# mfkiwl/msckf_stereo_c

Hardware: AMD Instinct MI355X
Metric: stereo frames/sec/node on EuRoC-shape input; ATE RMSE vs CPU ref (higher is better)
Workload: dtype f64

## Files before the change

msckf_stereo_c_amd/csrc/hip/ekf_kernels.hip:

```cpp
#include <mutex>
#include <type_traits>
#include "ekf_device.h"
#include "chol_block.h"

#define WG 256

__device__ __forceinline__ double wave_sum(double v) {
    for (int off = 32; off > 0; off >>= 1) v += __shfl_xor(v, off);
    return v;
}

__device__ __forceinline__ double block_sum(double v, double *s_red) {
    v = wave_sum(v);
    const int nw = blockDim.x >> 6;
    __syncthreads();
    if ((threadIdx.x & 63) == 0) s_red[threadIdx.x >> 6] = v;
    __syncthreads();
    double t = 0;
    for (int i = 0; i < nw; ++i) t += s_red[i];
    return t;
}

__device__ __forceinline__ void quat_to_rot(const double *q, double *R) {
    const double x = q[0], y = q[1], z = q[2], w = q[3];
    const double a = 2 * w * w - 1, tw = 2 * w;
    R[0] = a + 2 * x * x;        R[1] = tw * z + 2 * x * y;   R[2] = -tw * y + 2 * x * z;
    R[3] = -tw * z + 2 * y * x;  R[4] = a + 2 * y * y;        R[5] = tw * x + 2 * y * z;
    R[6] = tw * y + 2 * z * x;   R[7] = -tw * x + 2 * z * y;  R[8] = a + 2 * z * z;
}
__device__ __forceinline__ void mat3_mul(const double *A, const double *B, double *C) {
    for (int i = 0; i < 3; ++i) for (int j = 0; j < 3; ++j) C[3 * i + j] = A[3 * i] * B[j] + A[3 * i + 1] * B[3 + j] + A[3 * i + 2] * B[6 + j];
}
__device__ __forceinline__ void mat3_vec(const double *A, const double *v, double *o) {
    for (int i = 0; i < 3; ++i) o[i] = A[3 * i] * v[0] + A[3 * i + 1] * v[1] + A[3 * i + 2] * v[2];
}
__device__ __forceinline__ void mat3t_vec(const double *A, const double *v, double *o) {
    for (int i = 0; i < 3; ++i) o[i] = A[i] * v[0] + A[3 + i] * v[1] + A[6 + i] * v[2];
}

__device__ __forceinline__ void build_phi_q(const mskf_imu_step &st, const double *qc, double *sPhi, double *sA, double *sB) {
    constexpr int N = EKF_IMU_DIM;
    const int tid = threadIdx.x;
    for (int i = tid; i < N * N; i += WG) sA[i] = 0.0;
    __syncthreads();
    if (tid < 9) {
        const int r = tid / 3, c = tid % 3;
        const double g[3] = {st.gyro[0], st.gyro[1], st.gyro[2]}, a[3] = {st.acc[0], st.acc[1], st.acc[2]};
        const double skg[9] = {0, -g[2], g[1], g[2], 0, -g[0], -g[1], g[0], 0};
        const double ska[9] = {0, -a[2], a[1], a[2], 0, -a[0], -a[1], a[0], 0};
        double rs = 0;
        for (int k = 0; k < 3; ++k) rs += st.R_t[3 * r + k] * ska[3 * k + c];
        sA[r * N + c] = -skg[3 * r + c] * st.dt;
        sA[r * N + 3 + c] = (r == c ? -1.0 : 0.0) * st.dt;
        sA[(6 + r) * N + c] = -rs * st.dt;
        sA[(6 + r) * N + 9 + c] = -st.R_t[3 * r + c] * st.dt;
        sA[(12 + r) * N + 6 + c] = (r == c ? 1.0 : 0.0) * st.dt;
    }
    __syncthreads();
    for (int i = tid; i < N * N; i += WG) {
        const int r = i / N, c = i % N;
        double s2 = 0;
        for (int k = 0; k < N; ++k) s2 += sA[r * N + k] * sA[k * N + c];
        sB[i] = s2;
    }
    __syncthreads();
    for (int i = tid; i < N * N; i += WG) {
        const int r = i / N, c = i % N;
        double s3 = 0;
        for (int k = 0; k < N; ++k) s3 += sB[r * N + k] * sA[k * N + c];
        sPhi[i] = (r == c ? 1.0 : 0.0) + sA[i] + 0.5 * sB[i] + (1.0 / 6.0) * s3;
    }
    __syncthreads();
    if (tid < 9) {
        const int r = tid / 3, c = tid % 3;
        double a1u = 0, a2u = 0;
        for (int k = 0; k < 3; ++k) { a1u += sPhi[(6 + r) * N + k] * st.u[k]; a2u += sPhi[(12 + r) * N + k] * st.u[k]; }
        const double v1 = sPhi[(6 + r) * N + c] - (a1u - st.w1[r]) * st.s[c];
        const double v2 = sPhi[(12 + r) * N + c] - (a2u - st.w2[r]) * st.s[c];
        __builtin_amdgcn_wave_barrier();
        sPhi[(6 + r) * N + c] = v1;
        sPhi[(12 + r) * N + c] = v2;
        sPhi[r * N + c] = st.Phi00[3 * r + c];
    }
    __syncthreads();
    for (int i = tid; i < N * N; i += WG) {
        const int r = i / N, c = i % N;
        double q = 0;
        for (int k = 0; k < 12; ++k) q += sPhi[r * N + k] * qc[k / 3] * sPhi[c * N + k];
        sB[i] = q * st.dt;
    }
    __syncthreads();
    }

__global__ __launch_bounds__(WG) void k_ekf_propagate(const EkfStreamDev *streams) {
    const EkfStreamDev &S = streams[blockIdx.y];
    if (S.n_steps <= 0 && !S.J) return;
    double *P = S.P;
    const int d = S.d, ld = S.ld, N = EKF_IMU_DIM;
    __shared__ double sPhi[N * N], sQ[N * N], sP[N * N], sT[N * N], sTot[N * N], sJ[6 * N], sC[6 * N];
    const int tid = threadIdx.x;
    for (int i = tid; i < N * N; i += WG) { sP[i] = P[(size_t)(i / N) * ld + (i % N)]; sTot[i] = (i / N == i % N) ? 1.0 : 0.0; }
    for (int step = 0; step < S.n_steps; ++step) {
        __syncthreads();
        if (S.imu_steps && !S.PhiQ) {
            build_phi_q(S.imu_steps[step], S.qc, sPhi, sT, sQ);
        } else {
            const double *PhiQ = S.PhiQ + (size_t)step * 2 * N * N;
            for (int i = tid; i < N * N; i += WG) { sPhi[i] = PhiQ[i]; sQ[i] = PhiQ[N * N + i]; }
        }
        __syncthreads();
        double t0 = 0, t1 = 0;
        for (int i = tid; i < N * N; i += WG) {
            const int r = i / N, c = i % N;
            double s = 0, st2 = 0;
            for (int k = 0; k < N; ++k) { s += sPhi[r * N + k] * sP[k * N + c]; st2 += sPhi[r * N + k] * sTot[k * N + c]; }
            sT[i] = s;
            if (i < WG) t0 = st2; else t1 = st2;
        }
        __syncthreads();
        double x0 = 0, x1 = 0;
        for (int e = 0; e < 2; ++e) {
            const int i = tid + e * WG;
            if (i < N * N) {
                const int r = i / N, c = i % N;
                double s = 0, st = 0;
                for (int k = 0; k < N; ++k) { s += sT[r * N + k] * sPhi[c * N + k]; st += sT[c * N + k] * sPhi[r * N + k]; }
                const double v = ((s + sQ[r * N + c]) + (st + sQ[c * N + r])) * 0.5;
                if (e == 0) x0 = v; else x1 = v;
            }
        }
        __syncthreads();
        if (tid < N * N) { sP[tid] = x0; sTot[tid] = t0; }
        if (tid + WG < N * N) { sP[tid + WG] = x1; sTot[tid + WG] = t1; }
    }
    __syncthreads();
    if (S.J) for (int i = tid; i < 6 * N; i += WG) sJ[i] = S.J[i];
    __syncthreads();
    for (int c = tid; c < d; c += WG) {
        double col[N];
        if (c < N) { for (int k = 0; k < N; ++k) col[k] = sP[k * N + c]; }
        else {
            double old[N];
            for (int k = 0; k < N; ++k) old[k] = P[(size_t)k * ld + c];
            for (int r = 0; r < N; ++r) {
                double s = 0;
                for (int k = 0; k < N; ++k) s += sTot[r * N + k] * old[k];
                col[r] = s;
            }
            if (S.n_steps > 0) for (int r = 0; r < N; ++r) { P[(size_t)r * ld + c] = col[r]; P[(size_t)c * ld + r] = col[r]; }
        }
        if (S.J) {
            for (int r = 0; r < 6; ++r) {
                double s = 0;
                for (int k = 0; k < N; ++k) s += sJ[r * N + k] * col[k];
                P[(size_t)(d + r) * ld + c] = s;
                P[(size_t)c * ld + (d + r)] = s;
                if (c < N) sC[r * N + c] = s;
            }
        }
    }
    for (int i = tid; i < N * N; i += WG) P[(size_t)(i / N) * ld + (i % N)] = sP[i];
    if (S.J) {
        __syncthreads();
        if (tid < 36) {
            const int r = tid / 6, c = tid % 6;
            double s = 0, st = 0;
            for (int k = 0; k < N; ++k) { s += sC[r * N + k] * sJ[c * N + k]; st += sC[c * N + k] * sJ[r * N + k]; }
            P[(size_t)(d + r) * ld + (d + c)] = (s + st) / 2.0;
        }
    }
}

__global__ __launch_bounds__(WG) void k_ekf_augment(const EkfStreamDev *streams) {
    const EkfStreamDev &S = streams[blockIdx.y];
    if (!S.J) return;
    double *P = S.P;
    const int d = S.d, ld = S.ld, N = EKF_IMU_DIM;
    __shared__ double sJ[6 * N], sC[6 * N];
    const int tid = threadIdx.x;
    for (int i = tid; i < 6 * N; i += WG) sJ[i] = S.J[i];
    __syncthreads();
    for (int c = tid; c < d; c += WG) {
        double col[N];
        for (int k = 0; k < N; ++k) col[k] = P[(size_t)k * ld + c];
        for (int r = 0; r < 6; ++r) {
            double s = 0;
            for (int k = 0; k < N; ++k) s += sJ[r * N + k] * col[k];
            P[(size_t)(d + r) * ld + c] = s;
            P[(size_t)c * ld + (d + r)] = s;
            if (c < N) sC[r * N + c] = s;
        }
    }
    __syncthreads();
    if (tid < 36) {
        const int r = tid / 6, c = tid % 6;
        double s = 0, st = 0;
        for (int k = 0; k < N; ++k) { s += sC[r * N + k] * sJ[c * N + k]; st += sC[c * N + k] * sJ[r * N + k]; }
        P[(size_t)(d + r) * ld + (d + c)] = (s + st) / 2.0;
    }
}

__global__ __launch_bounds__(WG) void k_ekf_remove_clone(const EkfStreamDev *streams) {
    const EkfStreamDev &S = streams[blockIdx.y];
    if (S.remove_index < 0 || !S.P_dst) return;
    const int d = S.d, ld = S.ld;
    const int s0 = EKF_IMU_DIM + 6 * S.remove_index;
    const int s1 = S.remove_index2 >= 0 ? EKF_IMU_DIM + 6 * S.remove_index2 : (1 << 30);
    const int dn = d - (S.remove_index2 >= 0 ? 12 : 6);
    for (int idx = blockIdx.x * WG + threadIdx.x; idx < dn * dn; idx += gridDim.x * WG) {
        const int i = idx / dn, j = idx - i * dn;
        int si = i < s0 ? i : i + 6; if (si >= s1) si += 6;
        int sj = j < s0 ? j : j + 6; if (sj >= s1) sj += 6;
        S.P_dst[(size_t)i * ld + j] = S.P[(size_t)si * ld + sj];
    }
}

__global__ void k_ekf_posvar(const EkfStreamDev *streams, int n, double *out) {
    const int i = blockIdx.x * blockDim.x + threadIdx.x;
    if (i >= 3 * n) return;
    const EkfStreamDev &S = streams[i / 3];
    const int k = 12 + i % 3;
    out[i] = S.P[(size_t)k * S.ld + k];
}

__global__ void k_ekf_posvar_upd(const EkfStreamDev *streams, int n) {
    const int i = blockIdx.x * blockDim.x + threadIdx.x;
    if (i >= 3 * n) return;
    const EkfStreamDev &S = streams[i / 3];
    if (!S.pos_var_out || S.n_feat > 0) return;
    const int k = 12 + i % 3;
    S.pos_var_out[i % 3] = S.P[(size_t)k * S.ld + k];
}

#define MAX_CLONES_DEV 64

template <int NMEAS>
struct TriScratchT {
    double R[NMEAS][9];
    double t[NMEAS][3];
    double z[NMEAS][2];
};
typedef TriScratchT<2 * MAX_CLONES_DEV> TriScratch;
#define TRI_SMALL_CLONES 32

template <class TS>
__device__ bool triangulate_wave(const EkfStreamDev &S, const EkfFeatDev &F, TS &ts, double *pos_out) {
    const int lane = threadIdx.x & 63;
    const int n_meas = 2 * F.n_init;
    double R0[9], t0[3];
    {
        const mskf_clone_state &c = S.clones[S.obs_clone[F.init_start]];
        double Rw[9];
        quat_to_rot(c.q, Rw);
        for (int i = 0; i < 3; ++i) for (int j = 0; j < 3; ++j) R0[3 * i + j] = Rw[3 * j + i];
        t0[0] = c.p[0]; t0[1] = c.p[1]; t0[2] = c.p[2];
    }
    double Rinv[9], tinv[3];
    for (int i = 0; i < 3; ++i) for (int j = 0; j < 3; ++j) Rinv[3 * i + j] = S.R_c0_c1[3 * j + i];
    { double tmp[3]; mat3_vec(Rinv, S.t_c0_c1, tmp); tinv[0] = -tmp[0]; tinv[1] = -tmp[1]; tinv[2] = -tmp[2]; }
    for (int m = lane; m < n_meas; m += 64) {
        const int o = F.init_start + (m >> 1);
        const mskf_clone_state &c = S.clones[S.obs_clone[o]];
        double Rw[9], Rc[9], tc[3];
        quat_to_rot(c.q, Rw);
        for (int i = 0; i < 3; ++i) for (int j = 0; j < 3; ++j) Rc[3 * i + j] = Rw[3 * j + i];
        tc[0] = c.p[0]; tc[1] = c.p[1]; tc[2] = c.p[2];
        if (m & 1) {
            double R2[9], t2[3];
            mat3_mul(Rc, Rinv, R2);
            mat3_vec(Rc, tinv, t2);
            for (int i = 0; i < 9; ++i) Rc[i] = R2[i];
            for (int i = 0; i < 3; ++i) tc[i] = t2[i] + tc[i];
        }
        double Rt[9], dt[3] = {t0[0] - tc[0], t0[1] - tc[1], t0[2] - tc[2]};
        for (int i = 0; i < 3; ++i) for (int j = 0; j < 3; ++j) Rt[3 * i + j] = Rc[3 * j + i];
        mat3_mul(Rt, R0, ts.R[m]);
        mat3_vec(Rt, dt, ts.t[m]);
        ts.z[m][0] = S.obs_z[4 * o + ((m & 1) ? 2 : 0)];
        ts.z[m][1] = S.obs_z[4 * o + ((m & 1) ? 3 : 1)];
    }
    __builtin_amdgcn_wave_barrier();
    __threadfence_block();
    double sol[3];
    {
        const double *Rl = ts.R[n_meas - 1], *tl = ts.t[n_meas - 1];
        const double z1[2] = {ts.z[0][0], ts.z[0][1]}, z2[2] = {ts.z[n_meas - 1][0], ts.z[n_meas - 1][1]};
        double v[3] = {z1[0], z1[1], 1.0}, m[3];
        mat3_vec(Rl, v, m);
        const double A0 = m[0] - z2[0] * m[2], A1 = m[1] - z2[1] * m[2];
        const double b0 = z2[0] * tl[2] - tl[0], b1 = z2[1] * tl[2] - tl[1];
        const double depth = (A0 * b0 + A1 * b1) / (A0 * A0 + A1 * A1);
        const double p0 = z1[0] * depth, p1 = z1[1] * depth, p2 = depth;
        sol[0] = p0 / p2; sol[1] = p1 / p2; sol[2] = 1.0 / p2;
    }
    auto cost_of = [&](const double *x) {
        double e = 0;
        for (int m = lane; m < n_meas; m += 64) {
            const double *R = ts.R[m], *t = ts.t[m];
            const double h0 = R[0] * x[0] + R[1] * x[1] + R[2] + x[2] * t[0];
            const double h1 = R[3] * x[0] + R[4] * x[1] + R[5] + x[2] * t[1];
            const double h2 = R[6] * x[0] + R[7] * x[1] + R[8] + x[2] * t[2];
            const double d0 = h0 / h2 - ts.z[m][0], d1 = h1 / h2 - ts.z[m][1];
            e += d0 * d0 + d1 * d1;
        }
        return wave_sum(e);
    };
    double lambda = 1e-3;
    int inner = 0, outer = 0;
    bool reduced = false;
    double delta_norm = 0;
    double total_cost = cost_of(sol);
    do {
        double A[6] = {0, 0, 0, 0, 0, 0}, b[3] = {0, 0, 0};
        for (int m = lane; m < n_meas; m += 64) {
            const double *R = ts.R[m], *t = ts.t[m];
            const double h1 = R[0] * sol[0] + R[1] * sol[1] + R[2] + sol[2] * t[0];
            const double h2 = R[3] * sol[0] + R[4] * sol[1] + R[5] + sol[2] * t[1];
            const double h3 = R[6] * sol[0] + R[7] * sol[1] + R[8] + sol[2] * t[2];
            double W[3][3];
            for (int i = 0; i < 3; ++i) { W[i][0] = R[3 * i]; W[i][1] = R[3 * i + 1]; W[i][2] = t[i]; }
            double J0[3], J1[3];
            for (int j = 0; j < 3; ++j) {
                J0[j] = 1 / h3 * W[0][j] - h1 / (h3 * h3) * W[2][j];
                J1[j] = 1 / h3 * W[1][j] - h2 / (h3 * h3) * W[2][j];
            }
            const double r0 = h1 / h3 - ts.z[m][0], r1 = h2 / h3 - ts.z[m][1];
            const double e = sqrt(r0 * r0 + r1 * r1);
            const double w = (e <= 0.01) ? 1.0 : sqrt(2.0 * 0.01 / e);
            const double ws = (w == 1) ? 1.0 : w * w;
            A[0] += ws * (J0[0] * J0[0] + J1[0] * J1[0]); A[1] += ws * (J0[0] * J0[1] + J1[0] * J1[1]);
            A[2] += ws * (J0[0] * J0[2] + J1[0] * J1[2]); A[3] += ws * (J0[1] * J0[1] + J1[1] * J1[1]);
            A[4] += ws * (J0[1] * J0[2] + J1[1] * J1[2]); A[5] += ws * (J0[2] * J0[2] + J1[2] * J1[2]);
            b[0] += ws * (J0[0] * r0 + J1[0] * r1); b[1] += ws * (J0[1] * r0 + J1[1] * r1); b[2] += ws * (J0[2] * r0 + J1[2] * r1);
        }
        for (int i = 0; i < 6; ++i) A[i] = wave_sum(A[i]);
        for (int i = 0; i < 3; ++i) b[i] = wave_sum(b[i]);
        do {
            const double a00 = A[0] + lambda, a01 = A[1], a02 = A[2], a11 = A[3] + lambda, a12 = A[4], a22 = A[5] + lambda;
            double delta[3] = {0, 0, 0};
            const double l00 = sqrt(a00);
// ... 682 lines not shown
```

msckf_stereo_c_amd/csrc/hip/ekf_linalg.hip:

```cpp
#include <mutex>
#include <type_traits>
#include "ekf_device.h"
#include "ekf_cap.h"
#include "chol_block.h"

typedef double v4f64 __attribute__((ext_vector_type(4)));

#define QR_BIAS_LIMIT 1e-6
__device__ __forceinline__ bool ekf_mode_direct(int qr_mode, int stacked, int na) { return (qr_mode == 0 || qr_mode == 3) && stacked <= na; }
__device__ __forceinline__ bool ekf_mode_householder(int qr_mode) { return qr_mode == 2 || qr_mode == 3; }
__device__ __forceinline__ bool ekf_direct_wanted(const EkfStreamDev &S) { return ekf_mode_direct(S.qr_mode, S.rows_out[0], S.rows_out[2]); }
__device__ __forceinline__ bool ekf_skip_gram(const EkfStreamDev &S) { return ekf_mode_householder(S.qr_mode) || ekf_direct_wanted(S); }
__device__ __forceinline__ bool ekf_direct(const EkfStreamDev &S) { return (S.rows_out[3] & 4) != 0; }
#define EKF_ROUTE_PAIRS 1
#define EKF_ROUTE_WAVE 2
#define EKF_ROUTE_SMALL 4

enum { GM_GRAM = 0, GM_T = 1, GM_S2 = 2, GM_PUPD = 3 };

template <int MODE> struct GemmTraits;
template <> struct GemmTraits<GM_GRAM> { static constexpr bool TA = true,  SYM = true,  KMIN_I = false, KMIN_J = false; };
template <> struct GemmTraits<GM_T>    { static constexpr bool TA = true,  SYM = false, KMIN_I = true,  KMIN_J = false; };
template <> struct GemmTraits<GM_S2>   { static constexpr bool TA = false, SYM = true,  KMIN_I = false, KMIN_J = true;  };
template <> struct GemmTraits<GM_PUPD> { static constexpr bool TA = true,  SYM = true,  KMIN_I = false, KMIN_J = false; };
// ... 194 lines not shown
            ss = qr_lane_sum<Q>(ss);
            const double x0 = Rat(k, k);
            if (ss < 1e-200 || ss < 1e-40 * (x0 * x0)) continue;
            const double nrm = sqrt(x0 * x0 + ss);
            const double alpha = x0 > 0.0 ? -nrm : nrm;
            const double v0 = x0 - alpha;
            const double beta = 2.0 / (v0 * v0 + ss);
            for (int j = k + 1 + g; j < n1; j += ng) {
                double bj[RL];
                double dot = 0.0;
#pragma unroll
                for (int i = 0; i < RL; ++i) { bj[i] = own[i * n1 + j]; dot += bk[i] * bj[i]; }
                const double rkj = Rat(k, j);
                const double t = beta * (qr_lane_sum<Q>(dot) + v0 * rkj);
#pragma unroll
                for (int i = 0; i < RL; ++i) own[i * n1 + j] = bj[i] - t * bk[i];
                if (q == 0) Rat(k, j) = rkj - t * v0;
            }
            __syncthreads();
            if (tid == 0) Rat(k, k) = alpha;
        }
    }
    __syncthreads();
}
template <class ColOf, class RAt>
__device__ __forceinline__ void tsqr_quads(const EkfStreamDev &S, int n1, int K, ColOf colOf, RAt Rat, double *sB, int room) {
    if (room >= 48 * n1) tsqr_wide<4, 12>(S, n1, K, colOf, Rat, sB);
    else if (room >= 32 * n1) tsqr_wide<4, 8>(S, n1, K, colOf, Rat, sB);
    else tsqr_wide<4, 4>(S, n1, K, colOf, Rat, sB);
}

__device__ __forceinline__ int ekf_compress_entry(const EkfStreamDev &S, int *s_w ) {
    const int na = S.rows_out[2], me = S.rows_out[1], d = S.d, ld = S.ld;
    if (na <= 0) { if (threadIdx.x == 0) S.rows_out[3] = 0; return 1; }
    if (ekf_direct_wanted(S)) {
        int *rowidx = S.act + ld;
        const int tid = threadIdx.x, lane = tid & 63, wave = tid >> 6, nw = (int)blockDim.x >> 6;
        int base = 0;
        for (int r0 = 0; r0 < me; r0 += (int)blockDim.x) {
            const int r = r0 + tid;
            const bool on = r < me && S.rowmask[r] != 0ULL;
            const unsigned long long b = __ballot(on);
            if (lane == 0) s_w[wave] = __popcll(b);
            __syncthreads();
            int off = base, tot = 0;
            for (int w = 0; w < nw; ++w) { const int c = s_w[w]; if (w < wave) off += c; tot += c; }
            if (on && off + __popcll(b & ((1ULL << lane) - 1ULL)) < ld) rowidx[off + __popcll(b & ((1ULL << lane) - 1ULL))] = r;
            base += tot;
            __syncthreads();
        }
        __threadfence_block();
        __syncthreads();
        for (int i = tid; i < base; i += (int)blockDim.x) S.T[(size_t)i * ld + d] = S.Hs[(size_t)rowidx[i] * ld + d];
        if (tid == 0) { S.rows_out[3] = 4; S.rows_out[4] = base; }
        return 1;
    }
    return ekf_skip_gram(S) ? 2 : 0;
}
template <class RAt>
__device__ __forceinline__ void ekf_compress_exit(const EkfStreamDev &S, bool gram_done, int diag, RAt Rat, double *sB, int room) {
    const int na = S.rows_out[2], n1 = na + 1, K = S.rows_out[1], d = S.d, ld = S.ld;
    const int tid = threadIdx.x, nth = blockDim.x;
    const bool need = ekf_mode_householder(S.qr_mode) || (S.qr_mode == 0 && (!gram_done || (diag & 2)));
    if (!need) { if (tid == 0) S.rows_out[3] = diag; return; }
    __syncthreads();
    for (int e = tid; e < n1 * n1; e += nth) { const int k = e / n1, j = e - k * n1; if (j >= k) Rat(k, j) = 0.0; }
    const int *act = S.act;
    tsqr_quads(S, n1, K, [=](int c, int &col, int &clone) { col = c < na ? act[c] : d; clone = c < na ? (col - EKF_IMU_DIM) / 6 : -1; }, Rat, sB, room);
    for (int e = tid; e < na * na; e += nth) {
        const int i = e / na, j = e - i * na;
        if (j <= i) S.S[(size_t)i * ld + j] = Rat(j, i);
    }
    for (int k = tid; k < na; k += nth) S.T[(size_t)k * ld + d] = Rat(k, na);
    if (tid == 0) S.rows_out[3] = diag | 1;
}

#define TQ_THREADS 512
__device__ __forceinline__ double tq_rows_sum(double v) {
    {
        const unsigned long long b = (unsigned long long)__double_as_longlong(v);
        const auto lo = __builtin_amdgcn_permlane16_swap((unsigned)b, (unsigned)b, false, false), hi = __builtin_amdgcn_permlane16_swap((unsigned)(b >> 32), (unsigned)(b >> 32), false, false);
        v = __longlong_as_double((long long)(((unsigned long long)hi[0] << 32) | lo[0])) + __longlong_as_double((long long)(((unsigned long long)hi[1] << 32) | lo[1]));
    }
    {
        const unsigned long long b = (unsigned long long)__double_as_longlong(v);
        const auto lo = __builtin_amdgcn_permlane32_swap((unsigned)b, (unsigned)b, false, false), hi = __builtin_amdgcn_permlane32_swap((unsigned)(b >> 32), (unsigned)(b >> 32), false, false);
        v = __longlong_as_double((long long)(((unsigned long long)hi[0] << 32) | lo[0])) + __longlong_as_double((long long)(((unsigned long long)hi[1] << 32) | lo[1]));
    }
    return v;
}
__device__ __forceinline__ double tq_rcp(double x) {
    double r = __builtin_amdgcn_rcp(x);
    r = __builtin_fma(__builtin_fma(-x, r, 1.0), r, r);
    r = __builtin_fma(__builtin_fma(-x, r, 1.0), r, r);
    return r;
}
template <int C, bool FIRST> __device__ __forceinline__ void tq_fmac_bcast(double &acc, double x, double a) {
    if (FIRST) asm("s_nop 4\n\tv_fmac_f64_dpp %0, %1, %2 row_newbcast:%3 row_mask:0xf bank_mask:0xf" : "+v"(acc) : "v"(x), "v"(a), "n"(C));
    else asm("v_fmac_f64_dpp %0, %1, %2 row_newbcast:%3 row_mask:0xf bank_mask:0xf" : "+v"(acc) : "v"(x), "v"(a), "n"(C));
}
template <int RL, int I = 0> struct TqDot {
    static __device__ __forceinline__ void run(double (&p)[4], const double (&vr)[RL / 16], const double (&bc)[RL]) {
        tq_fmac_bcast<I % 16, I == 0>(p[I & 3], vr[I / 16], bc[I]);
        TqDot<RL, I + 1>::run(p, vr, bc);
    }
};
template <int RL> struct TqDot<RL, RL> { static __device__ __forceinline__ void run(double (&)[4], const double (&)[RL / 16], const double (&)[RL]) {} };
template <int RL, int I = 0> struct TqAxpy {
    static __device__ __forceinline__ void run(double (&bc)[RL], const double (&vr)[RL / 16], double ntt) {
        tq_fmac_bcast<I % 16, I == 0>(bc[I], vr[I / 16], ntt);
        TqAxpy<RL, I + 1>::run(bc, vr, ntt);
    }
};
template <int RL> struct TqAxpy<RL, RL> { static __device__ __forceinline__ void run(double (&)[RL], const double (&)[RL / 16], double) {} };
template <int RL>
__device__ __forceinline__ void tq_form_reflector(const double (&bc)[RL], double x0, double *sVs, int *sFlag_s, double *Rkk, int r) {
    double p0 = 0.0, p1 = 0.0, p2 = 0.0, p3 = 0.0;
#pragma unroll
    for (int i = 0; i < RL; i += 4) { p0 = __builtin_fma(bc[i], bc[i], p0); p1 = __builtin_fma(bc[i + 1], bc[i + 1], p1); p2 = __builtin_fma(bc[i + 2], bc[i + 2], p2); p3 = __builtin_fma(bc[i + 3], bc[i + 3], p3); }
    const double ss = tq_rows_sum((p0 + p1) + (p2 + p3));
    const bool skip = ss < 1e-200 || ss < 1e-40 * (x0 * x0);
    if (!skip) {
        const double n2 = __builtin_fma(x0, x0, ss);
        const double nrm = n2 * rsqrt_nr(n2);
        const double alpha = x0 > 0.0 ? -nrm : nrm;
        const double v0 = x0 - alpha;
        const double beta = 2.0 * tq_rcp(__builtin_fma(v0, v0, ss));
#pragma unroll
        for (int i = 0; i < RL; i += 2) *reinterpret_cast<double2 *>(sVs + r * RL + i) = make_double2(bc[i], bc[i + 1]);
        if (r == 0) { sVs[4 * RL] = v0; sVs[4 * RL + 1] = beta; *Rkk = alpha; }
    }
    if (r == 0) *sFlag_s = skip ? 0 : 1;
}
template <int RL, int NC>
__device__ __forceinline__ void tsqr_regs(const EkfStreamDev &S, int na, int K, double *Rg, double *sV, int *sFlag) {
    static_assert(RL % 16 == 0, "a DPP row holds the reflector's entries of its rows, 16 per register");
    constexpr int BR = 4 * RL, NW = TQ_THREADS / 64, SLAB = 16 * NW, VS = BR + 2, VR = RL / 16;
    const int n1 = na + 1, d = S.d, ld = S.ld;
    const int tid = threadIdx.x, lane = tid & 63, r = lane >> 4, c = lane & 15;
    const int wave = __builtin_amdgcn_readfirstlane(tid >> 6);
    int col[NC], clone[NC];
    bool has[NC];
#pragma unroll
    for (int t = 0; t < NC; ++t) {
        const int j = 16 * wave + c + SLAB * t;
        has[t] = j < n1;
        col[t] = j < na ? S.act[j] : d;
        clone[t] = j < na ? (col[t] - EKF_IMU_DIM) / 6 : -1;
    }
    for (int e = tid; e < n1 * n1; e += TQ_THREADS) { const int k = e / n1, j = e - k * n1; if (j >= k) Rg[(size_t)k * ld + j] = 0.0; }
    __syncthreads();
    for (int k0 = 0; k0 < K; k0 += BR) {
        double b[NC][RL];
#pragma unroll
        for (int i = 0; i < RL; ++i) {
            const int gk = k0 + r * RL + i;
            const unsigned long long rm = gk < K ? S.rowmask[gk] : 0ULL;
#pragma unroll
            for (int t = 0; t < NC; ++t) {
                const bool on = has[t] && (clone[t] < 0 ? rm != 0ULL : ((rm >> clone[t]) & 1ULL) != 0ULL);
                b[t][i] = on ? S.Hs[(size_t)gk * ld + col[t]] : 0.0;
            }
        }
        double ra[NC], rb[NC], rc[NC];
#pragma unroll
        for (int t = 0; t < NC; ++t) {
            const int j = 16 * wave + c + SLAB * t;
            ra[t] = has[t] ? Rg[j] : 0.0;
            rb[t] = has[t] && n1 > 1 ? Rg[(size_t)ld + j] : 0.0;
        }
        if (wave == 0 && c == 0) tq_form_reflector<RL>(b[0], ra[0], sV, sFlag, Rg, r);
        __syncthreads();
        for (int k = 0; k < n1; ++k) {
            const int s = k & 1;
            const double *vs = sV + s * VS;
            double vr[VR];
#pragma unroll
            for (int m = 0; m < VR; ++m) vr[m] = vs[r * RL + 16 * m + c];
            const double v0 = vs[BR], beta = vs[BR + 1];
            const bool live = __builtin_amdgcn_readfirstlane(sFlag[s]) != 0;
#pragma unroll
            for (int t = 0; t < NC; ++t) { const int j = 16 * wave + c + SLAB * t; rc[t] = (has[t] && k + 2 < n1) ? Rg[(size_t)(k + 2) * ld + j] : 0.0; }
            auto apply = [&](double (&bc)[RL], double rkj, int j, bool on) {
                double p[4] = {0.0, 0.0, 0.0, 0.0};
                TqDot<RL>::run(p, vr, bc);
                const double dot = tq_rows_sum((p[0] + p[1]) + (p[2] + p[3]));
                const double tt = on ? beta * __builtin_fma(v0, rkj, dot) : 0.0;
                TqAxpy<RL>::run(bc, vr, -tt);
                if (on && r == 0) Rg[(size_t)k * ld + j] = __builtin_fma(-tt, v0, rkj);
            };
            const int k1 = k + 1;
            const int w1 = (k1 & (SLAB - 1)) >> 4, c1 = k1 & 15, t1 = k1 / SLAB;
            const bool own_wave = k1 < n1 && wave == w1;
#pragma unroll
            for (int t = 0; t < NC; ++t) {
                if (own_wave && t1 == t) {
                    const int j = 16 * wave + c + SLAB * t;
                    if (live) apply(b[t], ra[t], j, has[t] && j > k);
                    if (c == c1) tq_form_reflector<RL>(b[t], rb[t], sV + (s ^ 1) * VS, sFlag + (s ^ 1), Rg + (size_t)k1 * ld + k1, r);
                }
            }
            if (live) {
#pragma unroll
                for (int t = 0; t < NC; ++t) {
                    const int j0 = 16 * wave + SLAB * t;
                    if (!(own_wave && t1 == t) && j0 + 15 > k && j0 < n1) apply(b[t], ra[t], j0 + c, has[t] && j0 + c > k);
                }
            }
#pragma unroll
            for (int t = 0; t < NC; ++t) { ra[t] = rb[t]; rb[t] = rc[t]; }
            __syncthreads();
        }
    }
}
template <int RL, int NC, class Load>
__device__ __forceinline__ void tsqr_wave(int n1, int n_blocks, int first, int stride, Load load, double *R, int ldr, double *sVw, int *sFlagw) {
    constexpr int BR = 4 * RL, VR = RL / 16;
    const int lane = threadIdx.x & 63, r = lane >> 4, c = lane & 15;
    for (int blk = first; blk < n_blocks; blk += stride) {
        double b[NC][RL];
#pragma unroll
        for (int i = 0; i < RL; ++i) {
#pragma unroll
            for (int t = 0; t < NC; ++t) b[t][i] = load(blk, r * RL + i, c + 16 * t);
        }
        for (int k = 0; k < n1; ++k) {
            const int tk = k >> 4, ck = k & 15;
#pragma unroll
            for (int t = 0; t < NC; ++t)
                if (tk == t && c == ck) tq_form_reflector<RL>(b[t], R[k * ldr + k], sVw, sFlagw, R + k * ldr + k, r);
            __builtin_amdgcn_wave_barrier();
            double vr[VR];
#pragma unroll
            for (int m = 0; m < VR; ++m) vr[m] = sVw[r * RL + 16 * m + c];
            const double v0 = sVw[BR], beta = sVw[BR + 1];
            const bool live = __builtin_amdgcn_readfirstlane(*sFlagw) != 0;
            if (live) {
#pragma unroll
                for (int t = 0; t < NC; ++t) {
                    if (16 * t + 15 > k && 16 * t < n1) {
                        const int j = c + 16 * t;
                        const bool on = j < n1 && j > k;
                        const double rkj = on ? R[k * ldr + j] : 0.0;
                        double p[4] = {0.0, 0.0, 0.0, 0.0};
                        TqDot<RL>::run(p, vr, b[t]);
                        const double dot = tq_rows_sum((p[0] + p[1]) + (p[2] + p[3]));
                        const double tt = on ? beta * __builtin_fma(v0, rkj, dot) : 0.0;
                        TqAxpy<RL>::run(b[t], vr, -tt);
                        if (on && r == 0) R[k * ldr + j] = __builtin_fma(-tt, v0, rkj);
                    }
                }
            }
            __builtin_amdgcn_wave_barrier();
        }
    }
}
template <int RL, int NC, int WPE>
__global__ __launch_bounds__(TQ_THREADS, WPE) void k_ekf_tsqr(const EkfStreamDev *streams, int do_cap) {
    const EkfStreamDev &S = streams[blockIdx.y];
    if (S.n_feat <= 0 || (S.route & EKF_ROUTE_SMALL)) return;
    if (!ekf_mode_householder(S.qr_mode)) return;
    if (do_cap) { (void)ekf_cap_local<TQ_THREADS>(S, true); __syncthreads(); }
    __shared__ int s_w[TQ_THREADS / 64];
    __shared__ __attribute__((aligned(16))) double sV[2 * (4 * RL + 2)];
    __shared__ int sFlag[2];
    if (ekf_compress_entry(S, s_w) != 2) return;
    const int na = S.rows_out[2], K = S.rows_out[1], d = S.d, ld = S.ld;
    const int tid = threadIdx.x;
    if (na + 1 > (TQ_THREADS / 4) * NC) { if (tid == 0) S.rows_out[3] = 0x80; return; }
    double *Rg = S.W;
    tsqr_regs<RL, NC>(S, na, K, Rg, sV, sFlag);
    for (int e = tid; e < na * na; e += TQ_THREADS) {
        const int i = e / na, j = e - i * na;
        if (j <= i) S.S[(size_t)i * ld + j] = Rg[(size_t)j * ld + i];
    }
    for (int k = tid; k < na; k += TQ_THREADS) S.T[(size_t)k * ld + d] = Rg[(size_t)k * ld + na];
    if (tid == 0) S.rows_out[3] = 1;
}

#define CHOLG_THREADS 512
__global__ __launch_bounds__(CHOLG_THREADS) void k_ekf_chol(const EkfStreamDev *streams, int which, int pan_rs) {
    const EkfStreamDev &S = streams[blockIdx.y];
    if (S.n_feat <= 0 || (S.route & EKF_ROUTE_SMALL)) return;
    int entry = 0;
    __shared__ int s_w[CHOLG_THREADS / 64];
    if (which == 0) {
        if (ekf_mode_householder(S.qr_mode)) return;
        entry = ekf_compress_entry(S, s_w);
        if (entry == 1) return;
    }
    const int n = which == 0 ? S.rows_out[2] : S.rows_out[4];
    const int nt = n + (which == 0 ? 1 : 0);
    const int lda = S.ld;
    double *A = which == 0 ? S.S : S.W;
    extern __shared__ double s_dyn[];
    double *sPanT = s_dyn;
    __shared__ double s_tol, s_mx[CHOLG_THREADS / 64];
    __shared__ int s_diag;
    __shared__ CholBlockShared s_cb;
    const int tid = threadIdx.x;
    if (tid == 0) s_diag = 0;
    for (int e = tid; e < LNB * pan_rs; e += CHOLG_THREADS) sPanT[e] = 0.0;
    if (which == 0) {
        double mx = 0;
        for (int i = tid; i < n; i += CHOLG_THREADS) mx = fmax(mx, A[(size_t)i * lda + i]);
        for (int off = 32; off > 0; off >>= 1) mx = fmax(mx, __shfl_xor(mx, off));
        if ((tid & 63) == 0) s_mx[tid >> 6] = mx;
        __syncthreads();
        if (tid == 0) { double m = 0; for (int i = 0; i < CHOLG_THREADS / 64; ++i) m = fmax(m, s_mx[i]); s_tol = m * (double)S.d * 1e-14; }
        __syncthreads();
        const double lam = s_tol;
        for (int i = tid; i < n; i += CHOLG_THREADS) A[(size_t)i * lda + i] += lam;
    }
    __syncthreads();
    chol_blocked_lds<CHOLG_THREADS / 64>(A, [lda](int i, int j) { return i * lda + j; }, n, nt, 0.0, sPanT, pan_rs, s_cb);
    if (which == 0) {
        int tiny = 0;
        for (int i = tid; i < n; i += CHOLG_THREADS) { const double l = A[(size_t)i * lda + i]; tiny += (l * l < 100.0 * s_tol) ? 1 : 0; }
        for (int o = 32; o > 0; o >>= 1) tiny += __shfl_xor(tiny, o);
        __shared__ int s_tiny[CHOLG_THREADS / 64];
        if ((tid & 63) == 0) s_tiny[tid >> 6] = tiny;
        __syncthreads();
        double pm = 0;
        for (int i = tid; i < n; i += CHOLG_THREADS) pm = fmax(pm, S.P[(size_t)S.act[i] * lda + S.act[i]]);
        for (int o = 32; o > 0; o >>= 1) pm = fmax(pm, __shfl_xor(pm, o));
        __syncthreads();
        if ((tid & 63) == 0) s_mx[tid >> 6] = pm;
        __syncthreads();
        if (tid == 0) {
            int t = 0; for (int i = 0; i < CHOLG_THREADS / 64; ++i) t += s_tiny[i];
            double p = 0; for (int i = 0; i < CHOLG_THREADS / 64; ++i) p = fmax(p, s_mx[i]);
            s_diag = (t << 8) | ((s_tol * p > QR_BIAS_LIMIT * S.sigma2) ? 2 : 0);
        }
        for (int k = tid; k < n; k += CHOLG_THREADS) S.T[(size_t)k * lda + S.d] = A[(size_t)n * lda + k];
        __syncthreads();
        double *Rg = S.W;
        ekf_compress_exit(S, true, s_diag, [=](int k, int j) -> double & { return Rg[(size_t)k * lda + j]; }, sPanT, LNB * pan_rs);
    }
}

#define CHOL_LDS_MAX_ROWS 181
#define CHOL_THREADS 512
#define CHOL_WAVES (CHOL_THREADS / 64)
#define CHOL_PAN_RS 192

__device__ __forceinline__ int pk(int i, int j) { return i * (i + 1) / 2 + j; }

__global__ __launch_bounds__(CHOL_THREADS) void k_ekf_chol_lds(const EkfStreamDev *streams, int which, int lds_doubles) {
    const EkfStreamDev &S = streams[blockIdx.y];
    if (S.n_feat <= 0 || (S.route & EKF_ROUTE_SMALL)) return;
    int entry = 0;
    __shared__ int s_w[CHOL_WAVES];
    if (which == 0) {
        if (ekf_mode_householder(S.qr_mode)) return;
        entry = ekf_compress_entry(S, s_w);
        if (entry == 1) return;
    }
    double *A = which == 0 ? S.S : S.W;
    const int off = 0, lda = S.ld;
    const int n = which == 0 ? S.rows_out[2] : S.rows_out[4];
    const int nt = n + (which == 0 ? 1 : 0);
    const bool semidef = which == 0;
    extern __shared__ double s_dyn[];
    double *sM = s_dyn;
    double *sPanT = s_dyn + nt * (nt + 1) / 2;
    __shared__ double s_tol, s_mx[CHOL_WAVES];
    __shared__ int s_diag;
    __shared__ CholBlockShared s_cb;
    const int tid = threadIdx.x, lane = tid & 63, wave = tid >> 6;
    if (tid == 0) s_diag = 0;
    auto Rl = [=](int k, int j) -> double & { return sM[k * nt - k * (k - 1) / 2 + (j - k)]; };
    const int room = lds_doubles - nt * (nt + 1) / 2;
    for (int i0 = wave * 8; i0 < nt; i0 += CHOL_WAVES * 8) {
        double v[8][3];
#pragma unroll
        for (int u = 0; u < 8; ++u) {
            const int i = i0 + u;
            const double *src = A + (size_t)(off + i) * lda + off;
// ... 114 lines not shown
                acc0 += l0[p] * y;
                acc1 += l1[p] * y;
            }
        }
        if (r8 < nb) sY[(ib + r8) * TS_COLS + c] -= acc0;
        if (r8 + 8 < nb) sY[(ib + r8 + 8) * TS_COLS + c] -= acc1;
        __syncthreads();
        if (tid < TS_COLS) {
            double x[TS_RB];
#pragma unroll
            for (int j = 0; j < TS_RB; ++j) {
                x[j] = 0.0;
                if (j < nb) {
                    double s2 = sY[(ib + j) * TS_COLS + tid];
                    const double *lj = sL + (size_t)j * (n + 1) + ib;
#pragma unroll
                    for (int cc = 0; cc < j; ++cc) s2 -= lj[cc] * x[cc];
                    x[j] = (lj[j] != 0.0) ? s2 / lj[j] : 0.0;
                    sY[(ib + j) * TS_COLS + tid] = x[j];
                }
            }
        }
    }
    __syncthreads();
    for (int e = tid; e < n * TS_COLS; e += 256) {
        const int i = e >> 5, cc = e & 31;
        if (c0 + cc < ncols) B[(size_t)i * ld + c0 + cc] = sY[e];
    }
}

#define SU_MAX_NA 24
#define SU_CH 128
__global__ __launch_bounds__(256) void k_ekf_small_update(const EkfStreamDev *streams) {
    const EkfStreamDev &S = streams[blockIdx.y];
    if (S.n_feat <= 0 || !(S.route & EKF_ROUTE_SMALL)) return;
    const EkfCapResult cap = ekf_cap_local(S, true);
    const int d = S.d, ld = S.ld, na = cap.na, n1 = na + 1, K = cap.end;
    const int tid = threadIdx.x;
    if (na <= 0 || na > SU_MAX_NA) {
        for (int c = tid; c < d; c += 256) S.delta_x[c] = 0.0;
        return;
    }
    extern __shared__ double s_dyn[];
    double *sT = s_dyn;
    double *sG = sT + (size_t)na * (d + 1);
    double *sS = sG + n1 * n1;
    double *sC = sS + na * na;
    __shared__ int s_col[SU_MAX_NA + 1], s_clone[SU_MAX_NA + 1];
    __shared__ double s_lam;
    if (tid < n1) {
        const int col = tid < na ? ekf_act_column(cap.clones, tid) : d;
        s_col[tid] = col;
        s_clone[tid] = tid < na ? (col - EKF_IMU_DIM) / 6 : -1;
    }
    __syncthreads();
    const bool hh_only = ekf_mode_householder(S.qr_mode);
    if (tid == 0) s_lam = 0.0;
    if (!hh_only) {
    const int np = n1 * (n1 + 1) / 2;
    const int groups = np <= 128 ? 256 / np : 1;
    int pi[2], pj[2], pg[2];
    double acc[2] = {0.0, 0.0};
    for (int q = 0; q < 2; ++q) {
        int p = tid + 256 * q, grp = 0;
        if (groups > 1) { grp = q == 0 ? tid / np : groups; p = tid - grp * np; }
        pg[q] = (groups > 1) ? (grp < groups ? grp : -1) : (p < np ? 0 : -1);
        if (pg[q] < 0) p = 0;
        int i = 0;
        while ((i + 1) * (i + 2) / 2 <= p) ++i;
        pi[q] = i; pj[q] = p - i * (i + 1) / 2;
    }
    for (int k0 = 0; k0 < K; k0 += SU_CH) {
        __syncthreads();
        for (int e = tid; e < SU_CH * n1; e += 256) {
            const int r = e / n1, c = e - r * n1, gk = k0 + r;
            double v = 0.0;
            if (gk < K) {
                const unsigned long long rm = S.rowmask[gk];
                const bool on = s_clone[c] < 0 ? rm != 0ULL : ((rm >> s_clone[c]) & 1ULL) != 0ULL;
                if (on) v = S.Hs[(size_t)gk * ld + s_col[c]];
            }
            sC[e] = v;
        }
        __syncthreads();
        for (int q = 0; q < 2; ++q) {
            if (pg[q] < 0) continue;
            double a = acc[q];
            for (int r = pg[q]; r < SU_CH; r += groups) a += sC[r * n1 + pi[q]] * sC[r * n1 + pj[q]];
            acc[q] = a;
        }
    }
    __syncthreads();
    if (groups > 1) {
        if (pg[0] >= 0) sC[pg[0] * np + (pi[0] * (pi[0] + 1) / 2 + pj[0])] = acc[0];
        __syncthreads();
        if (pg[0] == 0) {
            const int p = pi[0] * (pi[0] + 1) / 2 + pj[0];
            double t = 0.0;
            for (int g2 = 0; g2 < groups; ++g2) t += sC[g2 * np + p];
            sG[pi[0] * n1 + pj[0]] = t; sG[pj[0] * n1 + pi[0]] = t;
        }
    } else {
        for (int q = 0; q < 2; ++q)
            if (pg[q] >= 0) { sG[pi[q] * n1 + pj[q]] = acc[q]; sG[pj[q] * n1 + pi[q]] = acc[q]; }
    }
    __syncthreads();
    if (tid == 0) { double mx = 0; for (int i = 0; i < na; ++i) mx = fmax(mx, sG[i * n1 + i]); s_lam = mx * (double)d * 1e-14; }
    __syncthreads();
    if (tid < na) sG[tid * n1 + tid] += s_lam;
    __syncthreads();
    for (int k = 0; k < na; ++k) {
        const double pv = sG[k * n1 + k];
        const double inv = pv > 0.0 ? 1.0 / sqrt(pv) : 0.0;
        __syncthreads();
        if (tid >= k && tid < n1) sG[tid * n1 + k] = (tid == k) ? (pv > 0.0 ? sqrt(pv) : 0.0) : sG[tid * n1 + k] * inv;
        __syncthreads();
        for (int e = tid; e < (n1 - k - 1) * (n1 - k - 1); e += 256) {
            const int i = k + 1 + e / (n1 - k - 1), j = k + 1 + e % (n1 - k - 1);
            if (j <= i) sG[i * n1 + j] -= sG[i * n1 + k] * sG[j * n1 + k];
        }
        __syncthreads();
    }
    }
    {
        __shared__ int s_tiny, s_bias;
        if (tid == 0 && hh_only) { s_tiny = 0; s_bias = 0; }
        if (tid == 0 && !hh_only) {
            int t = 0;
            double pm = 0;
            for (int i = 0; i < na; ++i) {
                const double l = sG[i * n1 + i];
                t += (l * l < 100.0 * s_lam) ? 1 : 0;
                pm = fmax(pm, S.P[(size_t)s_col[i] * ld + s_col[i]]);
            }
            s_tiny = t;
            s_bias = (s_lam * pm > QR_BIAS_LIMIT * S.sigma2) ? 1 : 0;
        }
        __syncthreads();
        const int tiny = s_tiny;
        const bool need_qr = ekf_mode_householder(S.qr_mode) || (S.qr_mode == 0 && (cap.stacked <= na || s_bias));
        if (need_qr) {
            for (int e = tid; e < n1 * n1; e += 256) sG[e] = 0.0;
            __syncthreads();
            static_assert(SU_CH == 128 && SU_MAX_NA + 1 <= 32, "tsqr_wave<32, 2>: 128-row blocks, two 16-column slabs");
            {
                const int wv = __builtin_amdgcn_readfirstlane(tid >> 6);
                double *sRw = sC;
                double *sVq = (double *)(((uintptr_t)(sC + 3 * n1 * n1) + 15) & ~(uintptr_t)15);
                int *sFq = (int *)(sVq + 4 * 130);
                for (int e = tid; e < 3 * n1 * n1; e += 256) sRw[e] = 0.0;
                __syncthreads();
                const unsigned long long *rowmask = S.rowmask;
                const double *Hs = S.Hs;
                auto loadH = [&](int blk, int row, int col) -> double {
                    const int gk = blk * 128 + row;
                    if (gk >= K || col >= n1) return 0.0;
                    const unsigned long long rm = rowmask[gk];
                    const int cl = s_clone[col];
                    const bool on = cl < 0 ? rm != 0ULL : ((rm >> cl) & 1ULL) != 0ULL;
                    return on ? Hs[(size_t)gk * ld + s_col[col]] : 0.0;
                };
                double *Rmine = wv == 0 ? sG : sRw + (wv - 1) * n1 * n1;
                tsqr_wave<32, 2>(n1, (K + 127) / 128, wv, 4, loadH, Rmine, n1, sVq + wv * 130, sFq + wv);
                __syncthreads();
                if (wv == 0) {
                    auto loadR = [&](int, int row, int col) -> double {
                        if (row >= 3 * n1 || col >= n1) return 0.0;
                        const int w2 = row / n1, rr = row - w2 * n1;
                        return col >= rr ? sRw[(w2 * n1 + rr) * n1 + col] : 0.0;
                    };
                    tsqr_wave<32, 2>(n1, 1, 0, 1, loadR, sG, n1, sVq, sFq);
                }
                __syncthreads();
            }
            for (int e = tid; e < n1 * n1; e += 256) { const int i = e / n1, j = e - i * n1; if (j < i) sG[e] = sG[j * n1 + i]; }
            __syncthreads();
        }
        if (tid == 0) S.rows_out[3] = (tiny << 8) | (s_bias ? 2 : 0) | (need_qr ? 1 : 0);
    }
    const double *P = S.P;
    for (int c = tid; c < d; c += 256) {
        double pc[SU_MAX_NA];
#pragma unroll
        for (int k = 0; k < SU_MAX_NA; ++k) pc[k] = k < na ? P[(size_t)s_col[k] * ld + c] : 0.0;
#pragma unroll
        for (int i = 0; i < SU_MAX_NA; ++i) {
            if (i < na) {
                double t = 0.0;
#pragma unroll
                for (int k = i; k < SU_MAX_NA; ++k) if (k < na) t += sG[k * n1 + i] * pc[k];
                sT[i * (d + 1) + c] = t;
            }
        }
    }
    if (tid < na) sT[tid * (d + 1) + d] = sG[na * n1 + tid];
    __syncthreads();
    for (int e = tid; e < na * na; e += 256) {
        const int i = e / na, j = e - i * na;
        if (j > i) continue;
        double t = 0.0;
        for (int k = j; k < na; ++k) t += sT[i * (d + 1) + s_col[k]] * sG[k * n1 + j];
        if (i == j) t += S.sigma2;
        sS[i * na + j] = t; sS[j * na + i] = t;
    }
    __syncthreads();
    for (int k = 0; k < na; ++k) {
        const double pv = sS[k * na + k];
        const double inv = pv > 0.0 ? 1.0 / sqrt(pv) : 0.0;
        __syncthreads();
        if (tid >= k && tid < na) sS[tid * na + k] = (tid == k) ? (pv > 0.0 ? sqrt(pv) : 0.0) : sS[tid * na + k] * inv;
        __syncthreads();
        for (int e = tid; e < (na - k - 1) * (na - k - 1); e += 256) {
            const int i = k + 1 + e / (na - k - 1), j = k + 1 + e % (na - k - 1);
            if (j <= i) sS[i * na + j] -= sS[i * na + k] * sS[j * na + k];
        }
        __syncthreads();
    }
    for (int c = tid; c <= d; c += 256) {
        double y[SU_MAX_NA];
#pragma unroll
        for (int i = 0; i < SU_MAX_NA; ++i) {
            y[i] = 0.0;
            if (i >= na) continue;
            double t = sT[i * (d + 1) + c];
#pragma unroll
            for (int k = 0; k < i; ++k) t -= sS[i * na + k] * y[k];
            const double l = sS[i * na + i];
            y[i] = l != 0.0 ? t / l : 0.0;
            sT[i * (d + 1) + c] = y[i];
        }
    }
    __syncthreads();
    for (int e = tid; e < na * (d + 1); e += 256) {
        const int k = e / (d + 1), c = e - k * (d + 1);
        S.T[(size_t)k * ld + c] = sT[e];
    }
}

extern "C" {
void ekf_launch_gemm(const EkfStreamDev *d, int n, int mode, int max_mn, hipStream_t st) {
    const int t = (max_mn + GT - 1) / GT;
    const dim3 grid(t * t + (mode == GM_PUPD ? t : 0), n);
    switch (mode) {
        case GM_GRAM: hipLaunchKernelGGL(k_ekf_gemm<GM_GRAM>, grid, dim3(256), 0, st, d); break;
        case GM_T:    hipLaunchKernelGGL(k_ekf_gemm<GM_T>, grid, dim3(256), 0, st, d); break;
        case GM_S2:   hipLaunchKernelGGL(k_ekf_gemm<GM_S2>, grid, dim3(256), 0, st, d); break;
        default:      hipLaunchKernelGGL(k_ekf_gemm<GM_PUPD>, grid, dim3(256), 0, st, d); break;
    }
}
void ekf_launch_tsqr(const EkfStreamDev *d, int n, int max_d, int do_cap, hipStream_t st) {
    const int n1 = max_d - EKF_IMU_DIM + 1;
    if (n1 <= 2 * (TQ_THREADS / 4)) hipLaunchKernelGGL((k_ekf_tsqr<32, 2, 2>), dim3(1, n), dim3(TQ_THREADS), 0, st, d, do_cap);
    else hipLaunchKernelGGL((k_ekf_tsqr<16, 4, 2>), dim3(1, n), dim3(TQ_THREADS), 0, st, d, do_cap);
}
void ekf_launch_chol(const EkfStreamDev *d, int n, int which, int max_d, hipStream_t st) {
    const int nt = max_d - EKF_IMU_DIM + 1;
    if (nt <= CHOL_LDS_MAX_ROWS) {
        static std::once_flag attr_once;
    std::call_once(attr_once, []() { (void)hipFuncSetAttribute(reinterpret_cast<const void *>(k_ekf_chol_lds), hipFuncAttributeMaxDynamicSharedMemorySize,
                                      (int)(((size_t)CHOL_LDS_MAX_ROWS * (CHOL_LDS_MAX_ROWS + 1) / 2 + (size_t)CHOL_PAN_RS * LNB) * sizeof(double))); });
        const size_t lds = ((size_t)nt * (nt + 1) / 2 + (size_t)CHOL_PAN_RS * LNB) * sizeof(double);
        hipLaunchKernelGGL(k_ekf_chol_lds, dim3(1, n), dim3(CHOL_THREADS), lds, st, d, which, (int)(lds / sizeof(double)));
        return;
    }
    const int pan_rs = (nt + 15) / 16 * 16;
    hipLaunchKernelGGL(k_ekf_chol, dim3(1, n), dim3(CHOLG_THREADS), (size_t)LNB * pan_rs * sizeof(double), st, d, which, pan_rs);
}
void ekf_launch_small_update(const EkfStreamDev *d, int n, int max_d, hipStream_t st) {
    const size_t lds = ((size_t)SU_MAX_NA * (max_d + 1) + (SU_MAX_NA + 1) * (SU_MAX_NA + 1) + SU_MAX_NA * SU_MAX_NA + SU_CH * (SU_MAX_NA + 1)) * sizeof(double);
    static std::once_flag attr_once;
    std::call_once(attr_once, []() {
        hipFuncAttributes fa;
        size_t stat = 4096;
        if (hipFuncGetAttributes(&fa, reinterpret_cast<const void *>(k_ekf_small_update)) == hipSuccess) stat = fa.sharedSizeBytes;
        if (hipFuncSetAttribute(reinterpret_cast<const void *>(k_ekf_small_update), hipFuncAttributeMaxDynamicSharedMemorySize, (int)(160 * 1024 - stat)) != hipSuccess) (void)hipGetLastError();
    });
    hipLaunchKernelGGL(k_ekf_small_update, dim3(1, n), dim3(256), lds, st, d);
}
int ekf_small_update_max_na(void) { return SU_MAX_NA; }
void ekf_launch_trsm(const EkfStreamDev *d, int n, int max_d, hipStream_t st) {
    const int strips = (max_d + 1 + TS_COLS - 1) / TS_COLS;
    const int max_n = max_d > EKF_IMU_DIM ? max_d - EKF_IMU_DIM : 1;
    const size_t lds = (size_t)(TS_RB * (max_n + 1) + (size_t)max_n * TS_COLS) * sizeof(double);
    static std::once_flag attr_once;
    std::call_once(attr_once, []() { (void)hipFuncSetAttribute(reinterpret_cast<const void *>(k_ekf_trsm), hipFuncAttributeMaxDynamicSharedMemorySize, 160 * 1024); });
    hipLaunchKernelGGL(k_ekf_trsm, dim3(strips, n), dim3(256), lds, st, d);
}
}
```

Measured before the change: 99470.

## Fuse Jacobian augment into propagation column loop and batch unconditional H loads in QR

The propagation kernel now accumulates the 6-row clone Jacobian product on the fly while each propagated column entry is computed. This drops the intermediate col[N] array and the separate pass over it. The TSQR loaders now fetch whole 32-row blocks at once: row masks first, then unconditional Hs loads with clamped row indices, then masking. This lets the loads issue back to back instead of being serialized behind branches. An empty asm offset trick keeps the shared-memory bases in vector registers, probably to steer code generation, at the cost of more register pressure from the larger per-thread arrays.

```diff
diff --git a/msckf_stereo_c_amd/csrc/hip/ekf_kernels.hip b/msckf_stereo_c_amd/csrc/hip/ekf_kernels.hip
--- a/msckf_stereo_c_amd/csrc/hip/ekf_kernels.hip
+++ b/msckf_stereo_c_amd/csrc/hip/ekf_kernels.hip
@@ -137,25 +137,31 @@
     if (S.J) for (int i = tid; i < 6 * N; i += WG) sJ[i] = S.J[i];
     __syncthreads();
     for (int c = tid; c < d; c += WG) {
-        double col[N];
-        if (c < N) { for (int k = 0; k < N; ++k) col[k] = sP[k * N + c]; }
-        else {
+        int o = 0;
+        asm volatile("" : "+v"(o));
+        const double *tot = sTot + o, *jj = sJ + o;
+        const bool aug = S.J != nullptr;
+        double jacc[6] = {0.0, 0.0, 0.0, 0.0, 0.0, 0.0};
+        if (c < N) {
+            for (int k = 0; k < N; ++k) {
+                const double v = sP[k * N + c];
+                if (aug) for (int r = 0; r < 6; ++r) jacc[r] += jj[r * N + k] * v;
+            }
+        } else {
             double old[N];
             for (int k = 0; k < N; ++k) old[k] = P[(size_t)k * ld + c];
             for (int r = 0; r < N; ++r) {
                 double s = 0;
-                for (int k = 0; k < N; ++k) s += sTot[r * N + k] * old[k];
-                col[r] = s;
-            }
-            if (S.n_steps > 0) for (int r = 0; r < N; ++r) { P[(size_t)r * ld + c] = col[r]; P[(size_t)c * ld + r] = col[r]; }
-        }
-        if (S.J) {
+                for (int k = 0; k < N; ++k) s += tot[r * N + k] * old[k];
+                if (S.n_steps > 0) { P[(size_t)r * ld + c] = s; P[(size_t)c * ld + r] = s; }
+                if (aug) for (int q = 0; q < 6; ++q) jacc[q] += jj[q * N + r] * s;
+            }
+        }
+        if (aug) {
             for (int r = 0; r < 6; ++r) {
-                double s = 0;
-                for (int k = 0; k < N; ++k) s += sJ[r * N + k] * col[k];
-                P[(size_t)(d + r) * ld + c] = s;
-                P[(size_t)c * ld + (d + r)] = s;
-                if (c < N) sC[r * N + c] = s;
+                P[(size_t)(d + r) * ld + c] = jacc[r];
+                P[(size_t)c * ld + (d + r)] = jacc[r];
+                if (c < N) sC[r * N + c] = jacc[r];
             }
         }
     }
@@ -181,11 +187,14 @@
     for (int i = tid; i < 6 * N; i += WG) sJ[i] = S.J[i];
     __syncthreads();
     for (int c = tid; c < d; c += WG) {
+        int o = 0;
+        asm volatile("" : "+v"(o));
+        const double *jj = sJ + o;
         double col[N];
         for (int k = 0; k < N; ++k) col[k] = P[(size_t)k * ld + c];
         for (int r = 0; r < 6; ++r) {
             double s = 0;
-            for (int k = 0; k < N; ++k) s += sJ[r * N + k] * col[k];
+            for (int k = 0; k < N; ++k) s += jj[r * N + k] * col[k];
             P[(size_t)(d + r) * ld + c] = s;
             P[(size_t)c * ld + (d + r)] = s;
             if (c < N) sC[r * N + c] = s;
diff --git a/msckf_stereo_c_amd/csrc/hip/ekf_linalg.hip b/msckf_stereo_c_amd/csrc/hip/ekf_linalg.hip
--- a/msckf_stereo_c_amd/csrc/hip/ekf_linalg.hip
+++ b/msckf_stereo_c_amd/csrc/hip/ekf_linalg.hip
@@ -370,14 +370,21 @@
     __syncthreads();
     for (int k0 = 0; k0 < K; k0 += BR) {
         double b[NC][RL];
+        unsigned long long rm[RL];
+#pragma unroll
+        for (int i = 0; i < RL; ++i) { const int gk = k0 + r * RL + i; rm[i] = gk < K ? S.rowmask[gk] : 0ULL; }
 #pragma unroll
         for (int i = 0; i < RL; ++i) {
-            const int gk = k0 + r * RL + i;
-            const unsigned long long rm = gk < K ? S.rowmask[gk] : 0ULL;
+            const int gk = min(k0 + r * RL + i, K - 1);
+#pragma unroll
+            for (int t = 0; t < NC; ++t) b[t][i] = S.Hs[(size_t)gk * ld + col[t]];
+        }
+#pragma unroll
+        for (int i = 0; i < RL; ++i) {
 #pragma unroll
             for (int t = 0; t < NC; ++t) {
-                const bool on = has[t] && (clone[t] < 0 ? rm != 0ULL : ((rm >> clone[t]) & 1ULL) != 0ULL);
-                b[t][i] = on ? S.Hs[(size_t)gk * ld + col[t]] : 0.0;
+                const bool on = has[t] && (clone[t] < 0 ? rm[i] != 0ULL : ((rm[i] >> clone[t]) & 1ULL) != 0ULL);
+                b[t][i] = on ? b[t][i] : 0.0;
             }
         }
         double ra[NC], rb[NC], rc[NC];
@@ -437,11 +444,7 @@
     const int lane = threadIdx.x & 63, r = lane >> 4, c = lane & 15;
     for (int blk = first; blk < n_blocks; blk += stride) {
         double b[NC][RL];
-#pragma unroll
-        for (int i = 0; i < RL; ++i) {
-#pragma unroll
-            for (int t = 0; t < NC; ++t) b[t][i] = load(blk, r * RL + i, c + 16 * t);
-        }
+        load(blk, r * RL, c, b);
         for (int k = 0; k < n1; ++k) {
             const int tk = k >> 4, ck = k & 15;
 #pragma unroll
@@ -862,22 +865,43 @@
                 __syncthreads();
                 const unsigned long long *rowmask = S.rowmask;
                 const double *Hs = S.Hs;
-                auto loadH = [&](int blk, int row, int col) -> double {
-                    const int gk = blk * 128 + row;
-                    if (gk >= K || col >= n1) return 0.0;
-                    const unsigned long long rm = rowmask[gk];
-                    const int cl = s_clone[col];
-                    const bool on = cl < 0 ? rm != 0ULL : ((rm >> cl) & 1ULL) != 0ULL;
-                    return on ? Hs[(size_t)gk * ld + s_col[col]] : 0.0;
+                auto loadH = [&](int blk, int row0, int c, double (&bb)[2][32]) {
+                    unsigned long long rm[32];
+                    int colx[2], cl[2];
+                    bool has[2];
+#pragma unroll
+                    for (int t = 0; t < 2; ++t) { const int col = c + 16 * t; has[t] = col < n1; colx[t] = s_col[has[t] ? col : 0]; cl[t] = s_clone[has[t] ? col : 0]; }
+#pragma unroll
+                    for (int i = 0; i < 32; ++i) { const int gk = blk * 128 + row0 + i; rm[i] = gk < K ? rowmask[gk] : 0ULL; }
+#pragma unroll
+                    for (int i = 0; i < 32; ++i) {
+                        const int gk = min(blk * 128 + row0 + i, K - 1);
+#pragma unroll
+                        for (int t = 0; t < 2; ++t) bb[t][i] = Hs[(size_t)gk * ld + colx[t]];
+                    }
+#pragma unroll
+                    for (int i = 0; i < 32; ++i) {
+#pragma unroll
+                        for (int t = 0; t < 2; ++t) {
+                            const bool on = has[t] && (cl[t] < 0 ? rm[i] != 0ULL : ((rm[i] >> cl[t]) & 1ULL) != 0ULL);
+                            bb[t][i] = on ? bb[t][i] : 0.0;
+                        }
+                    }
                 };
                 double *Rmine = wv == 0 ? sG : sRw + (wv - 1) * n1 * n1;
                 tsqr_wave<32, 2>(n1, (K + 127) / 128, wv, 4, loadH, Rmine, n1, sVq + wv * 130, sFq + wv);
                 __syncthreads();
                 if (wv == 0) {
-                    auto loadR = [&](int, int row, int col) -> double {
-                        if (row >= 3 * n1 || col >= n1) return 0.0;
-                        const int w2 = row / n1, rr = row - w2 * n1;
-                        return col >= rr ? sRw[(w2 * n1 + rr) * n1 + col] : 0.0;
+                    auto loadR = [&](int, int row0, int c, double (&bb)[2][32]) {
+#pragma unroll
+                        for (int i = 0; i < 32; ++i) {
+#pragma unroll
+                            for (int t = 0; t < 2; ++t) {
+                                const int row = row0 + i, col = c + 16 * t;
+                                const int w2 = row / n1, rr = row - w2 * n1;
+                                bb[t][i] = (row < 3 * n1 && col < n1 && col >= rr) ? sRw[(w2 * n1 + rr) * n1 + col] : 0.0;
+                            }
+                        }
                     };
                     tsqr_wave<32, 2>(n1, 1, 0, 1, loadR, sG, n1, sVq, sFq);
                 }
```

Result: faster. 101,500 (median of 6 runs) (+2.1%).
